# ayildiri/polymer-chemprop

Hardware: AMD Instinct MI355X
Metric: edges/sec MPN forward, batch=64 polymer graphs, depth=3 hidden=300 (higher is better)
Workload: dtype fp32; 1 GPU; MPNEncoder.forward on synthetic polymer batches of 64 graphs (avg E=6164 directed edges), depth=3, hidden=300, 8 resident batches cycled per rank; global_batch=64, depth=3, hidden=300, parallelism=dp1 (independent graphs, no collective in the forward), streams=3

## Files before the change

polymer-chemprop_amd/csrc/common.hpp:

```cpp
#pragma once
#include <hip/hip_runtime.h>
#include <stdint.h>

#include <type_traits>

namespace wd {

typedef float floatx16 __attribute__((ext_vector_type(16)));

enum Act : int { ACT_RELU = 0, ACT_LEAKY = 1, ACT_PRELU = 2, ACT_TANH = 3, ACT_SELU = 4, ACT_ELU = 5,
                 ACT_IDENTITY = 6 };

constexpr float SELU_ALPHA = 1.6732632423543772848170429916717f;
constexpr float SELU_SCALE = 1.0507009873554804934193349852946f;

__device__ __forceinline__ float act_fwd(int act, float z, float slope) {
    switch (act) {
    case ACT_RELU: return z < 0.f ? 0.f : z;
    case ACT_LEAKY: return z > 0.f ? z : 0.1f * z;
    case ACT_PRELU: return z > 0.f ? z : slope * z;
    case ACT_TANH: return tanhf(z);
    case ACT_SELU: return z > 0.f ? SELU_SCALE * z : SELU_SCALE * (SELU_ALPHA * expm1f(z));
    case ACT_ELU: return z > 0.f ? z : expm1f(z);
    default: return z;
// ... 37 lines not shown
    }
}

__device__ __forceinline__ float dropout_scale(uint64_t seed, uint32_t layer, uint32_t row, uint32_t col, float p) {
    uint64_t x = seed ^ (0x9E3779B97F4A7C15ull * (uint64_t)(layer + 1));
    x ^= ((uint64_t)row << 32) | col;
    x += 0x9E3779B97F4A7C15ull;
    x = (x ^ (x >> 30)) * 0xBF58476D1CE4E5B9ull;
    x = (x ^ (x >> 27)) * 0x94D049BB133111EBull;
    x ^= x >> 31;
    const float u = (float)(uint32_t)(x >> 40) * (1.0f / 16777216.0f);
    return u >= p ? 1.0f / (1.0f - p) : 0.0f;
}

#ifndef WD_STAMPS
#define WD_STAMPS 0
#endif
#if WD_STAMPS
constexpr int WD_STAMP_SLOTS = 16, WD_STAMP_WG = 8192;
__device__ uint64_t g_wd_stamps[WD_STAMP_WG * WD_STAMP_SLOTS];
__device__ __forceinline__ void wd_stamp(int slot) {
    const uint64_t t = __builtin_amdgcn_s_memrealtime();
    if (threadIdx.x == 0 && blockIdx.x < WD_STAMP_WG)
        __hip_atomic_store(&g_wd_stamps[blockIdx.x * WD_STAMP_SLOTS + slot], t, __ATOMIC_RELAXED, __HIP_MEMORY_SCOPE_AGENT);
}
constexpr int WD_LSTAMP_WG = 512;
__device__ uint64_t g_wd_lstamps[WD_LSTAMP_WG * 16 * 8];
__device__ uint64_t g_wd_estamps[WD_STAMP_WG * 8];
__device__ __forceinline__ void wd_estamp(int slot) {
    const uint64_t t = __builtin_amdgcn_s_memrealtime();
    if (threadIdx.x == 0 && blockIdx.x < WD_STAMP_WG)
        __hip_atomic_store(&g_wd_estamps[blockIdx.x * 8 + slot], t, __ATOMIC_RELAXED, __HIP_MEMORY_SCOPE_AGENT);
}
__device__ __forceinline__ void wd_lstamp(int chunk, int slot) {
    const uint64_t t = __builtin_amdgcn_s_memtime();
    if ((threadIdx.x & 63) == 0 && blockIdx.x < WD_LSTAMP_WG && chunk < 16)
        __hip_atomic_store(&g_wd_lstamps[(blockIdx.x * 16 + chunk) * 8 + slot], t, __ATOMIC_RELAXED, __HIP_MEMORY_SCOPE_AGENT);
}
#else
__device__ __forceinline__ void wd_stamp(int) {}
__device__ __forceinline__ void wd_estamp(int) {}
__device__ __forceinline__ void wd_lstamp(int, int) {}
#endif

__device__ __forceinline__ float4 f4zero() { return make_float4(0.f, 0.f, 0.f, 0.f); }

__device__ __forceinline__ void fma4(float4 &acc, float c, const float4 &v) {
    acc.x = fmaf(c, v.x, acc.x);
    acc.y = fmaf(c, v.y, acc.y);
    acc.z = fmaf(c, v.z, acc.z);
    acc.w = fmaf(c, v.w, acc.w);
}

__device__ __forceinline__ float4 ld4(const float *p) { return *reinterpret_cast<const float4 *>(p); }
__device__ __forceinline__ void st4(float *p, const float4 &v) { *reinterpret_cast<float4 *>(p) = v; }

__device__ __forceinline__ int xcd_tile(int b, int ntiles) {
    const int base = ntiles >> 3, rem = ntiles & 7;
    const int x = b & 7, local = b >> 3;
    return x * base + (x < rem ? x : rem) + local;
}

constexpr int WD_MULTI = 8;
template <typename T, int NJ = WD_MULTI> struct Multi {
    T p[NJ];
    int t0[NJ + 1];
    int n;
};
template <typename T, int NJ>
__device__ __forceinline__ const T &multi_pick(const Multi<T, NJ> &M, int g, int &tile) {
    int j = 0;
    while (j + 1 < M.n && g >= M.t0[j + 1]) ++j;
    tile = g - M.t0[j];
    return M.p[j];
// ... 4 lines not shown
```

polymer-chemprop_amd/csrc/fused_mp.hpp:

```cpp
#pragma once
#include "gemm_x6.hpp"
#include "kernels.hpp"
#include "wdmpnn.h"

namespace wd {


constexpr int BLK_BONDS = 128, BLK_ATOMS = 64;
constexpr int BLK_MOLS = 64;
constexpr int ELLW = 8;
static_assert(ELLW % 4 == 0, "ELL rows of whole 4-byte index words and float4 weight groups");

struct EllRow {
    uint32_t ix[ELLW / 4];
    float w[ELLW];
};
__device__ __forceinline__ EllRow ell_zero() {
    EllRow e;
    for (int k = 0; k < ELLW / 4; ++k) e.ix[k] = 0;
    for (int k = 0; k < ELLW; ++k) e.w[k] = 0.f;
    return e;
}
__device__ __forceinline__ EllRow ell_load(const uint8_t *idx, const float *coef, size_t row) {
    EllRow e;
// ... 676 lines not shown
            const int v = tid + NT * u, lb = v / U8, c = 8 * (v % U8);
            if (lb >= ((B.bn + 15) & ~15)) break;
            h2_store8(prs, h2_blk_off<BLK_BONDS>(lb, n0 + c), BLK_BONDS * 64, ym[u][0], ym[u][1], s);
        }
        wd_estamp(7);
    } else {
        publish_max(mx, P.amax + (size_t)blk * P.n_tiles + nt, red);
    }
    if constexpr (EO_LAST) {
        __syncthreads();
        eo_half();
    }
}

constexpr int WO_MAXK = 160;

struct WoReadoutP {
    const uint8_t *fa; int kpa; int kca;
    int kcw;
    const uint8_t *ag; int kp;
    const uint8_t *wo;
    const float *bias;
    const int32_t *blocks;
    const float *w_atoms; const int32_t *mol_start, *mol_size; const float *xn;
    int agg; float norm; const float *zero_vec;
    int act; const float *slope; float p_drop; uint64_t seed; uint32_t layer;
    float *out; int ncols;
    int n_tiles;
    const float *eo;
    int Hk, ldeo;
    float *zosave;
    const uint8_t *apairs; const uint32_t *a_amax; int a_nw, a_g;
    const uint8_t *woh; const uint32_t *wo_amax;
};

template <int BN> struct WoWaves;
template <> struct WoWaves<64> { static constexpr int WM = 4, WN = 2; };
template <> struct WoWaves<80> { static constexpr int WM = 2, WN = 5; };

template <int BN, int CPS, int NJ = WD_MULTI, bool PAIRS = false>
__global__ __launch_bounds__(PAIRS ? 512 : 64 * WoWaves<BN>::WM * WoWaves<BN>::WN, PAIRS ? 4 : 1) void wo_readout_kernel(const Multi<WoReadoutP, NJ> MP) {
    constexpr int BM = BLK_ATOMS, LDC = BN + 4, WM = PAIRS ? 4 : WoWaves<BN>::WM, WN = PAIRS ? 1 : WoWaves<BN>::WN;
    constexpr int NT = PAIRS ? 512 : 64 * WM * WN;
    constexpr int WS = 2;
    constexpr int EPI_BYTES = (BM * LDC + BM + 3 * BLK_MOLS + BN) * 4;
    constexpr int LDS_BYTES = PAIRS ? (h2p_lds_bytes<BM, BN>() > EPI_BYTES ? h2p_lds_bytes<BM, BN>() : EPI_BYTES)
                                    : WS * CPS * x6_stage_bytes<BM, BN>();
    __shared__ __attribute__((aligned(16))) uint8_t lds[LDS_BYTES];
    int tile;
    const WoReadoutP &P = multi_pick(MP, xcd_tile(blockIdx.x, gridDim.x), tile);
    const int blk = tile / P.n_tiles, nt = tile % P.n_tiles, n0 = nt * BN;
    BlockRow B = PAIRS ? BlockRow{} : load_block(P.blocks, blk);
    const int tid = threadIdx.x;
    X6Operands O{};
    O.a0 = P.fa; O.nkc0 = P.kpa >> 5; O.kc0 = P.kca;
    O.a1 = P.ag; O.nkc1 = P.kp >> 5; O.kc1 = P.kp >> 5;
    O.rb = blk;
    O.a_rows = B.an;
    O.b = P.wo + ((size_t)nt * (P.kcw + (P.kp >> 5)) + (P.kcw - P.kca)) * (3 * BN * 64);
    constexpr int C4 = BN / 4;
    static_assert((PAIRS || NT % C4 == 0) && BM <= NT, "one bias group per thread, one atom weight per thread");
    int nm = min(B.mh - B.ml, BLK_MOLS);
    if (P.zosave && blk == 0 && tid < BN / 4) st4(P.zosave + n0 + 4 * tid, f4zero());
    float4 bb = f4zero();
    float watom = 0.f, mxn = 0.f;
    int mstart = 0, msize = 0;
    constexpr int EPU = (BM * C4 + NT - 1) / NT;
    float4 eo[EPU];
    auto prefetch = [&](int phase) {
        if (phase != 0) return;
        if (!PAIRS || tid < C4) bb = ld4(P.bias + n0 + 4 * (tid % C4));
        if (tid < B.an) watom = P.w_atoms[B.as + tid];
#pragma unroll
        for (int j = 0; j < EPU; ++j) {
            const int v = tid + NT * j, la = v / C4, c = 4 * (v % C4);
            eo[j] = P.eo && v < BM * C4 && la < B.an ? ld4(P.eo + (size_t)(B.as + la) * P.ldeo + n0 + c) : f4zero();
        }
        if (tid < nm) {
            mstart = P.mol_start[B.ml + tid];
            msize = P.mol_size[B.ml + tid];
            mxn = P.xn[B.ml + tid];
        }
    };
    float *H = reinterpret_cast<float *>(lds);
    floatx4 acc[BM / WM / 16][BN / WN / 16];
    if constexpr (PAIRS) {
        auto rows = [&]() {
            B = load_block(P.blocks, blk);
            nm = min(B.mh - B.ml, BLK_MOLS);
            prefetch(0);
            return B.an;
        };
        uint32_t wom = 0;
        auto words = [&]() {
            wom = *P.wo_amax;
            return lane_word(P.a_amax + (size_t)blk * P.a_nw, P.a_nw);
        };
        int se;
        h2_mainloop_pairs<BM, BN>(P.apairs + (size_t)blk * (P.kp >> 5) * (2 * BM * 64),
                                  P.woh + (size_t)nt * (P.kp >> 5) * (2 * BN * 64), P.kp >> 5, rows, words, P.a_g, lds,
                                  acc, se);
        __syncthreads();
        if (threadIdx.x < 256)
            x6_acc_to_lds_scaled<BM, BN, 4, 1>(acc, H, se >= 0 ? __uint_as_float((uint32_t)(254 - se) << 23) : 1.f,
                                               h2_inv_scale(wom));
    } else {
        x6_mainloop<BM, BN, WM, WN, WS, CPS>(O, lds, acc, prefetch);
        __syncthreads();
        x6_acc_to_lds<BM, BN, WM, WN>(acc, H);
    }
    float *Wl = H + BM * LDC;
    float *Ml = Wl + BM;
    static_assert(EPI_BYTES <= LDS_BYTES, "readout staging fits");
    static_assert(BLK_MOLS <= NT, "one molecule per thread in the prefetch");
    if (tid < BM) Wl[tid] = watom;
    if (PAIRS && tid < C4) st4(Ml + 3 * BLK_MOLS + 4 * tid, bb);
    if (tid < nm) {
        Ml[tid] = __int_as_float(mstart);
        Ml[BLK_MOLS + tid] = __int_as_float(msize);
        Ml[2 * BLK_MOLS + tid] = mxn;
    }
    __syncthreads();
    with_act(P.act, [&](auto act_c) {
        constexpr int ACT = decltype(act_c)::value;
        const float slope = ACT == ACT_PRELU ? P.slope[0] : 0.f;
#pragma unroll
        for (int j = 0; j < EPU; ++j) {
            const int v = tid + NT * j;
            if (v >= BM * C4) break;
            const int la = v / C4, c = 4 * (v % C4);
            float4 hv = ld4(H + la * LDC + c);
            hv.x += eo[j].x; hv.y += eo[j].y; hv.z += eo[j].z; hv.w += eo[j].w;
            const float4 b4 = PAIRS ? ld4(Ml + 3 * BLK_MOLS + c) : bb;
            float z[4] = {hv.x + b4.x, hv.y + b4.y, hv.z + b4.z, hv.w + b4.w};
            if (P.zosave && la < B.an) st4(P.zosave + (size_t)(B.as + la) * P.Hk + n0 + c, make_float4(z[0], z[1], z[2], z[3]));
#pragma unroll
            for (int q = 0; q < 4; ++q) z[q] = act_fwd(ACT, z[q], slope);
            if (P.p_drop > 0.f && la < B.an)
#pragma unroll
                for (int q = 0; q < 4; ++q) z[q] *= dropout_scale(P.seed, P.layer, B.as + la, n0 + c + q, P.p_drop);
            st4(H + la * LDC + c, make_float4(z[0], z[1], z[2], z[3]));
        }
    });
    __syncthreads();
    constexpr int RP = 8;
    static_assert(NT % RP == 0 && 64 % RP == 0, "lane groups stay inside a wave");
    for (int t = tid; t < nm * BN * RP; t += NT) {
        const int part = t % RP, u = t / RP, im = u / BN, i = B.ml + im, cc = u % BN, col = n0 + cc;
        const int n = __float_as_int(Ml[BLK_MOLS + im]);
        float s = 0.f, wsum = 0.f;
        const int a0 = __float_as_int(Ml[im]) - B.as;
        for (int a = part; a < n; a += RP) {
            const float w = Wl[a0 + a];
            s = fmaf(w, H[(a0 + a) * LDC + cc], s);
            wsum += w;
        }
#pragma unroll
        for (int off = 1; off < RP; off <<= 1) {
            s += __shfl_xor(s, off, 64);
            wsum += __shfl_xor(wsum, off, 64);
        }
        if (part != 0 || col >= P.ncols) continue;
        float v;
        if (n == 0) {
            v = P.zero_vec[col];
        } else {
            const float m = P.agg == 0 ? s / wsum : (P.agg == 2 ? s / P.norm : s);
            v = Ml[2 * BLK_MOLS + im] * m;
        }
        P.out[(size_t)i * P.ncols + col] = v;
    }
}

}
```

polymer-chemprop_amd/csrc/gemm_x6.hpp:

```cpp
#pragma once
#include "gemm.hpp"
#include "planes.hpp"

#include <type_traits>

namespace wd {

#ifndef WD_STAMP_GEMM
#define WD_STAMP_GEMM 0
#endif

struct X6Params {
    const float *a0; int lda0; int ka0;
    const float *a1; int lda1; int ka1;
    const float *bf; int ldb;
    int M, N;
    int tiles_m, tiles_n;
    Epi epi;
    const uint32_t *a_words; int a_cv;
    const uint32_t *b_word;
};

template <int BM, int BK, bool H2 = false>
__global__ __launch_bounds__(4 * BM) void gemm_x6_kernel(X6Params P) {
// ... 796 lines not shown
        if (kc + H2_B_AHEAD < nchunks) issue_b(kc + H2_B_AHEAD);
        const uint8_t *st = lds + (kc % NA) * ASTAGE, *sb = lds + NA * ASTAGE + (kc % NB) * BSTAGE;
        dispatch_upto<TM>(na, [&](auto c) { compute_n(st, sb, c); });
        if (WD_STAMPS && wave == 0) {
            asm volatile("s_waitcnt lgkmcnt(0)" ::: "memory");
            wd_lstamp(kc, 3);
        }
    }
    __builtin_amdgcn_s_waitcnt(0x0070);
}

#ifndef WD_H2P_STAGES
#define WD_H2P_STAGES 3
#endif
constexpr int H2P_STAGES = WD_H2P_STAGES;
template <int BM, int BN>
constexpr int h2p_stage_bytes() { return 2 * BM * 64 + 2 * BN * 64; }
template <int BM, int BN>
constexpr int h2p_lds_bytes() { return H2P_STAGES * h2p_stage_bytes<BM, BN>(); }

#ifndef WD_H2P_FRAG
#define WD_H2P_FRAG 0
#endif
#ifndef WD_H2P_EARLY
#define WD_H2P_EARLY 0
#endif
#ifndef WD_H2P_UNIFORM
#define WD_H2P_UNIFORM 1
#endif
struct NoLoaderHook {
    __device__ void issue() {}
    __device__ void finish() {}
};
template <int BM, int BN, int FRAG = WD_H2P_FRAG, typename Rows, typename Words, typename LoaderHook = NoLoaderHook>
__device__ __forceinline__ void h2_mainloop_pairs(const uint8_t *a_src, const uint8_t *b_src, int nchunks, Rows &&rows,
                                                  Words &&words, int G, uint8_t *lds, floatx4 (&acc)[BM / 64][BN / 16],
                                                  int &se_out, LoaderHook &&lhook = LoaderHook()) {
    constexpr bool EARLY = WD_H2P_EARLY;
    static_assert(BM == 128 || BM == 64, "four consumer waves of BM / 4 rows");
    constexpr int RW = BM / 4, TM = RW / 16, TN = BN / 16;
    constexpr int APL = BM * 64, BPL = BN * 64, STAGE = h2p_stage_bytes<BM, BN>(), NS = H2P_STAGES;
    constexpr int AP = 2 * BM / 16, APW = AP / 4;
    constexpr int BP = 2 * BN / 16, BPW = (BP + 3) / 4;
    static_assert(AP % 4 == 0, "A pieces split evenly over the loader waves");
    const int tid = threadIdx.x, lane = tid & 63, wave = WD_H2P_UNIFORM ? __builtin_amdgcn_readfirstlane(tid >> 6) : tid >> 6, w4 = wave & 3;
    const int g = lane >> 4, i16 = lane & 15;
    const int roff = (NS - (nchunks - 1) % NS) % NS;
#pragma unroll
    for (int a = 0; a < TM; ++a)
#pragma unroll
        for (int b = 0; b < TN; ++b) acc[a][b] = floatx4{0.f, 0.f, 0.f, 0.f};
    if (wave >= 4) {
        int src[APW + BPW], dst[APW + BPW];
#pragma unroll
        for (int j = 0; j < APW; ++j) {
            const int c = 4 * j + w4, q = 64 * c + lane, p = q / (BM * 4), r = (q >> 2) % BM, sl = q & 3;
            src[j] = p * APL + r * 64 + 16 * (sl ^ ((r >> 1) & 3));
            dst[j] = 1024 * c;
        }
#pragma unroll
        for (int j = 0; j < BPW; ++j) {
            const int c = 4 * j + w4, q = 64 * c + lane, p = (q / (BN * 4)) % 2, r = (q >> 2) % BN, sl = q & 3;
            src[APW + j] = p * BPL + r * 64 + 16 * (sl ^ ((r >> 1) & 3));
            dst[APW + j] = 2 * APL + 1024 * c;
        }
        auto issue = [&](int kc, const bool (&on)[APW + BPW]) {
            uint8_t *st = lds + ((kc + roff) % NS) * STAGE;
            const uint8_t *ablk = a_src + (size_t)kc * (2 * APL), *bblk = b_src + (size_t)kc * (2 * BPL);
#pragma unroll
            for (int j = 0; j < APW; ++j)
                if (on[j]) glds16_untracked(ablk + src[j], st + dst[j]);
#pragma unroll
            for (int j = 0; j < BPW; ++j)
                if (on[APW + j]) glds16_untracked(bblk + src[APW + j], st + dst[APW + j]);
        };
        bool all[APW + BPW], on[APW + BPW];
#pragma unroll
        for (int j = 0; j < APW; ++j) all[j] = true;
#pragma unroll
        for (int j = 0; j < BPW; ++j) all[APW + j] = BP % 4 == 0 || 4 * j + w4 < BP;
        if constexpr (EARLY) {
#pragma unroll
            for (int c = 0; c < NS - 1; ++c)
                if (c < nchunks) issue(c, all);
            __builtin_amdgcn_sched_barrier(0);
        }
        const int a_rows = rows();
        int mine = 0;
#pragma unroll
        for (int j = 0; j < APW; ++j) {
            on[j] = 16 * ((4 * j + w4) % (BM / 16)) < a_rows;
            mine += on[j];
        }
#pragma unroll
        for (int j = 0; j < BPW; ++j) {
            on[APW + j] = all[APW + j];
            mine += on[APW + j];
        }
        mine = __builtin_amdgcn_readfirstlane(mine);
        if constexpr (!EARLY) {
#pragma unroll
            for (int c = 0; c < NS - 1; ++c)
                if (c < nchunks) issue(c, on);
        }
        lhook.issue();
        dispatch_upto<APW + BPW>(mine, [&](auto m_c) {
            constexpr int M = decltype(m_c)::value;
            for (int kc = 0; kc < nchunks; ++kc) {
                if (WD_STAMPS && wave == 4) wd_lstamp(kc, 4);
                if (nchunks - 1 - kc >= NS - 2) asm volatile("s_waitcnt vmcnt(%0)" ::"n"((NS - 2) * M) : "memory");
                else wait_vmcnt((nchunks - 1 - kc) * M);
                if (WD_STAMPS && wave == 4) wd_lstamp(kc, 5);
                __builtin_amdgcn_s_barrier();
                if (kc + NS - 1 < nchunks) issue(kc + NS - 1, on);
            }
        });
        __builtin_amdgcn_s_waitcnt(0x0070);
        lhook.finish();
        se_out = -1;
        return;
    }
    const int a_rows = rows();
    const uint32_t wv = words();
    int ao[TM], bo[TN];
#pragma unroll
    for (int a = 0; a < TM; ++a) ao[a] = x6_slot(RW * w4 + 16 * a + i16, g);
#pragma unroll
    for (int b = 0; b < TN; ++b) bo[b] = x6_slot(16 * b + i16, g);
    const int na = min(TM, max(0, (a_rows - RW * w4 + 15) >> 4));
    constexpr int BIG = 1 << 20;
    const int k0 = min((32 * lane) / G, 63), k1 = min((32 * lane + 16) / G, 63);
    const uint32_t lw0 = (uint32_t)__shfl((int)wv, k0, 64), lw1 = (uint32_t)__shfl((int)wv, k1, 64);
    const int s0 = lw0 ? h2_sexp(lw0) : BIG, s1 = lw1 ? h2_sexp(lw1) : BIG;
    const int cur = BIG - (int)wave_max_u32((uint32_t)(BIG - (lane < nchunks ? min(s0, s1) : BIG)));
    auto f16code = [&](int se) -> uint32_t {
        const int d = se - cur;
        return d > 24 ? 0u : (uint32_t)__builtin_bit_cast(unsigned short, (_Float16)__builtin_amdgcn_ldexpf(1.0f, -d));
    };
    const uint32_t fcode = f16code(s0) | (f16code(s1) << 16);
    const int fsh = lane < 32 ? 0 : 16;
    auto compute_n = [&](const uint8_t *st, const uint8_t *sb, auto na_c, _Float16 fl) {
        constexpr int NA = decltype(na_c)::value;
        constexpr int SCH = FRAG & 3, NB = SCH == 2 ? TN : 2;
        f16x8 af[TM][2], bq[NB][2];
#pragma unroll
        for (int p = 0; p < 2; ++p) {
#pragma unroll
            for (int a = 0; a < NA; ++a) {
                af[a][p] = *reinterpret_cast<const f16x8 *>(st + p * APL + ao[a]);
                af[a][p] = af[a][p] * fl;
            }
#pragma unroll
            for (int b = 0; b < (SCH == 2 ? TN : 1); ++b) bq[b][p] = *reinterpret_cast<const f16x8 *>(sb + p * BPL + bo[b]);
        }
#pragma unroll
        for (int b = 0; b < TN; ++b) {
            const int cb = SCH == 2 ? b : (b & 1);
            if constexpr (SCH == 1) {
                if (b + 1 < TN)
#pragma unroll
                    for (int p = 0; p < 2; ++p) bq[(b + 1) & 1][p] = *reinterpret_cast<const f16x8 *>(sb + p * BPL + bo[b + 1]);
                __builtin_amdgcn_sched_barrier(0);
// ... 106 lines not shown
```

polymer-chemprop_amd/csrc/wdmpnn.hip:

```cpp
#include <hip/hip_runtime.h>

#include <algorithm>
#include <array>
#include <cstdarg>
#include <cstdio>
#include <cstdlib>
#include <cmath>
#include <cstring>
#include <string>
#include <vector>

#include "feed.hpp"
#include "fused_mp.hpp"
#include "gemm.hpp"
#include "gemm_x6.hpp"
#include "graph_build.hpp"
#include "kernels.hpp"
#include "selfcheck.hpp"
#include "small_fwd.hpp"
#include "wdmpnn.h"

using namespace wd;

namespace {
// ... 14 lines not shown
#define WD_KERNELS_OK() WD_TRY(self_check_once())

#define WD_CHECK_LAUNCH(what)                                                                  \
    do {                                                                                       \
        hipError_t e_ = hipGetLastError();                                                     \
        if (e_ != hipSuccess) return fail(-(int)e_, "%s: %s", what, hipGetErrorString(e_));   \
    } while (0)
#define WD_TRY(x)             \
    do {                      \
        int rc_ = (x);        \
        if (rc_) return rc_;  \
    } while (0)

struct SelfCheck {
    int rc;
    std::string why;
    int n_host, n_dev;
};
const SelfCheck &self_check_result() {
    static const SelfCheck r = [] {
        SelfCheck c{};
        c.rc = code_object_check(reinterpret_cast<const void *>(&self_check_result), c.why, c.n_host, c.n_dev);
        return c;
    }();
    return r;
}
int self_check_once() {
    const SelfCheck &c = self_check_result();
    return c.rc ? fail(WD_ERR_UNSUPPORTED, "libwdmpnn self-check: %s", c.why.c_str()) : 0;
}

#ifndef WD_WO_PAIRS
#define WD_WO_PAIRS 1
#endif

#ifndef WD_FEED_EVENT_SYNC
#define WD_FEED_EVENT_SYNC hipEventBlockingSync
#endif

#ifndef WD_BWD_H2
#define WD_BWD_H2 1
#endif

inline int rup(int x, int m) { return (x + m - 1) / m * m; }


inline size_t align256(size_t x) { return (x + 255) & ~size_t(255); }
bool aligned16(const void *p) { return ((uintptr_t)p & 15) == 0; }

int ew_blocks(size_t total) {
    size_t b = (total + 255) / 256;
    if (b > 4096) b = 4096;
    if (b < 1) b = 1;
    return (int)b;
}

struct Variant {
    bool f32;
    bool one_launch;
    bool staged;
    bool pairs;
    bool pair_tiles;
    int stop;
    bool wo_dump;
};
Variant decode_variant(int v) {
// ... 645 lines not shown
    L.mol_start = take((size_t)c->n_mols * 4 + 4);
    L.mol_size = take((size_t)c->n_mols * 4 + 4);
    L.xn = take((size_t)c->n_mols * 4 + 4);
    L.b2revb = take((size_t)c->n_bonds * 4);
    L.blocks = take((size_t)c->n_blocks * 32 + 32);
    L.bond_blk_row = take((size_t)L.Rbp * 4);
    L.atom_blk_row = take((size_t)L.Vap * 4);
    L.bond_src_blk = take((size_t)L.Rbp);
    L.bond_tail = take((size_t)L.Rbp * 2);
    L.msg_ell_idx = take((size_t)L.Rbp * GB_ELLW);
    L.msg_ell_coef = take((size_t)L.Rbp * GB_ELLW * 4);
    L.agg_ell_idx = take((size_t)L.Vap * GB_ELLW);
    L.agg_ell_coef = take((size_t)L.Vap * GB_ELLW * 4);
    const int rows[4] = {c->n_bonds, c->n_atoms, c->n_bonds, c->n_bonds};
    const int nnz[4] = {c->nnz_msg, c->nnz_agg, c->nnz_msg, c->nnz_agg};
    for (int q = 0; q < 4; ++q) {
        L.csr[q][0] = take((size_t)(rows[q] + 1) * 4);
        L.csr[q][1] = take((size_t)(nnz[q] + GB_CSR_PAD) * 4);
        L.csr[q][2] = take((size_t)(nnz[q] + GB_CSR_PAD) * 4);
    }
    L.total = off;
    return 0;
}

struct FusedJob {
    const WdGraph *g;
    Dims D;
    FwdLayout L;
    char *ws;
    float *out;
};

template <typename T, typename Fill>
int launch_multi(const FusedJob *jobs, int n, int tiles_per_blk, Fill &&fill, Multi<T> &M) {
    M = Multi<T>{};
    M.n = n;
    int t = 0;
    for (int j = 0; j < n; ++j) {
        M.t0[j] = t;
        fill(M.p[j], jobs[j]);
        t += jobs[j].D.nblk * tiles_per_blk;
    }
    for (int j = n; j <= WD_MULTI; ++j) M.t0[j] = t;
    return t;
}
template <typename T>
Multi<T, 1> one_job(const Multi<T> &M) {
    Multi<T, 1> o{};
    o.p[0] = M.p[0]; o.t0[0] = M.t0[0]; o.t0[1] = M.t0[1]; o.n = 1;
    return o;
}
template <typename T, typename Launch>
void with_jobs(int n, const Multi<T> &M, Launch &&launch) {
    if (n == 1) launch(one_job(M), std::integral_constant<int, 1>{});
    else launch(M, std::integral_constant<int, WD_MULTI>{});
}

struct FusedCtx {
    const FusedJob *jobs;
    int n;
    const WdParams *p;
    const WdConfig *c;
    const PackLayout &PL;
    const char *pk;
    hipStream_t st;
    const Dims &D0;
    int Hk, BN;
    const float *W(size_t off) const { return (const float *)(pk + off); }
    static float *F(const FusedJob &J, size_t off) { return (float *)(J.ws + off); }
    static uint32_t *slot(const FusedJob &J, int t) { return (uint32_t *)(J.ws + J.L.amax[t & 1]); }
};

int fused_input(const FusedCtx &X) {
    const Dims &D0 = X.D0;
// ... 97 lines not shown
            Q.apairs = last && D0.wo_pairs ? (uint8_t *)(J.ws + J.L.Ab) : nullptr;
            Q.amax_out = X.slot(J, t);
        }
    }, M);
    auto go = [&](auto bn_c, auto last_c) {
        constexpr int BNc = decltype(bn_c)::value;
        constexpr bool LAST = decltype(last_c)::value;
        host_with_act(X.c->activation, [&](auto act_c) {
            constexpr int A = decltype(act_c)::value;
            if (D0.atom)
                hipLaunchKernelGGL((mp_layer_kernel<BNc, LAST, A, true, 1>), dim3(grid), dim3(MP_THREADS), 0, X.st, one_job(M));
            else with_jobs(X.n, M, [&](const auto &Mn, auto nj) {
                constexpr int NJ = decltype(nj)::value;
                if (BNc != 80 || !pairs)
                    hipLaunchKernelGGL((mp_layer_kernel<BNc, LAST, A, false, NJ>), dim3(grid), dim3(MP_THREADS), 0, X.st, Mn);
                else if constexpr (BNc == 80)
                    hipLaunchKernelGGL((mp_layer_kernel<BNc, LAST, A, false, NJ, true>), dim3(grid), dim3(MP_THREADS), 0, X.st, Mn);
            });
        });
    };
    using I80 = std::integral_constant<int, 80>;
    using I64 = std::integral_constant<int, 64>;
    if (BN == 80) { if (last) go(I80{}, std::true_type{}); else go(I80{}, std::false_type{}); }
    else { if (last) go(I64{}, std::true_type{}); else go(I64{}, std::false_type{}); }
    WD_CHECK_LAUNCH("mp_layer");
    return 0;
}

int fused_wo_readout(const FusedCtx &X) {
    const Dims &D0 = X.D0;
    const PackLayout &PL = X.PL;
    const int Hk = X.Hk, BN = X.BN;
    Multi<WoReadoutP> M;
    const int grid = launch_multi(X.jobs, X.n, Hk / BN, [&](WoReadoutP &R, const FusedJob &J) {
        const WdGraph *g = J.g;
        R.fa = g->f_atoms_blk_x6 ? (const uint8_t *)g->f_atoms_blk_x6 : (const uint8_t *)(J.ws + J.L.Ab);
        R.kpa = g->ld_atoms; R.kcw = J.D.Fak / 32;
        R.kca = D0.codes || J.D.atom ? 0 : R.kcw;
        R.eo = D0.codes ? X.F(J, J.L.Eo) : (J.D.atom ? X.F(J, J.L.In3) + 2 * Hk : nullptr); R.Hk = Hk;
        R.ldeo = J.D.atom ? 3 * Hk : Hk;
        R.ag = (const uint8_t *)(J.ws + J.L.Ab); R.kp = Hk;
        R.wo = (const uint8_t *)(X.pk + (BN == 80 ? PL.WoX80 : PL.WoX)); R.bias = X.W(PL.bo);
        R.blocks = g->blocks;
        R.w_atoms = g->w_atoms; R.mol_start = g->mol_start; R.mol_size = g->mol_size; R.xn = g->degree_of_polym;
        R.agg = X.c->aggregation; R.norm = X.c->aggregation_norm; R.zero_vec = X.p->zero_vec;
        R.act = X.c->activation; R.slope = X.p->prelu; R.p_drop = X.c->dropout; R.seed = X.c->seed; R.layer = J.D.T;
        R.out = J.out; R.ncols = J.D.H; R.n_tiles = Hk / BN;
        R.zosave = J.D.save ? X.F(J, J.L.Zo) : nullptr;
        if (D0.V.wo_dump && J.D.T == 3)
            R.zosave = D0.lay_pairs ? X.F(J, J.L.Mp[1]) : X.F(J, J.L.Zb[1]);
        if (D0.wo_pairs) {
            R.apairs = (const uint8_t *)(J.ws + J.L.Ab); R.a_amax = X.slot(J, J.D.T - 1); R.a_nw = Hk / BN; R.a_g = BN;
            R.woh = (const uint8_t *)(X.pk + PL.WoH); R.wo_amax = (const uint32_t *)(X.pk + PL.wo_amax) + 64;
        }
    }, M);
    if (grid <= 0) return 0;
    with_jobs(X.n, M, [&](const auto &Mn, auto nj) {
        constexpr int NJ = decltype(nj)::value;
        if (D0.wo_pairs)
            hipLaunchKernelGGL((wo_readout_kernel<80, 1, NJ, true>), dim3(grid), dim3(512), 0, X.st, Mn);
        else if (BN == 80)
            hipLaunchKernelGGL((wo_readout_kernel<80, NJ == 1 ? 1 : 2, NJ>), dim3(grid), dim3(64 * WoWaves<80>::WM * WoWaves<80>::WN), 0, X.st, Mn);
        else
            hipLaunchKernelGGL((wo_readout_kernel<64, 1, NJ>), dim3(grid), dim3(64 * WoWaves<64>::WM * WoWaves<64>::WN), 0, X.st, Mn);
    });
    WD_CHECK_LAUNCH("wo_readout");
    return 0;
}

int fused_forward(const FusedJob *jobs, int n, const WdParams *p, const WdConfig *c, const PackLayout &PL,
                  const char *pk, hipStream_t st) {
    if (n < 1 || n > WD_MULTI) return fail(WD_ERR_ARG, "fused forward: %d jobs per launch (1..%d)", n, WD_MULTI);
    const Dims &D0 = jobs[0].D;
    if (D0.atom && n > 1)
        return fail(WD_ERR_UNSUPPORTED, "fused forward: atom messages run one batch per launch");
    for (int j = 1; j < n; ++j) {
        const Dims &D = jobs[j].D;
        if (D.codes != D0.codes || D.Hk != D0.Hk || D.T != D0.T || D.atom != D0.atom || D.Fa != D0.Fa ||
            D.Fb != D0.Fb || D.save != D0.save || D.pairs != D0.pairs)
            return fail(WD_ERR_UNSUPPORTED, "fused forward: batches of one launch differ in layout");
    }
    const FusedCtx X{jobs, n, p, c, PL, pk, st, D0, D0.Hk, D0.bn};
    const int stop = D0.V.stop;
    WD_TRY(fused_input(X));
    if (D0.codes && stop == 1) return 0;
    for (int t = 1; t < D0.T; ++t) {
        if (t == 1) WD_TRY(record_prof(c, 0, 0, st));
        WD_TRY(fused_layer(X, t));
        if (t == D0.T - 1) WD_TRY(record_prof(c, 0, 1, st));
        if (stop == t + 1) return 0;
    }
    return fused_wo_readout(X);
// ... 35 lines not shown
int wdmpnn_abi_version(void) { return WDMPNN_ABI_VERSION; }

int wdmpnn_self_check(int32_t *n_host_kernels, int32_t *n_device_kernels) {
    const SelfCheck &c = self_check_result();
    if (n_host_kernels) *n_host_kernels = c.n_host;
    if (n_device_kernels) *n_device_kernels = c.n_dev;
    return self_check_once();
}

int wdmpnn_debug_fwd_offsets(const WdGraph *g, const WdParams *p, const WdConfig *c, size_t *out) {
    Dims D;
    WD_TRY(get_dims(g, p, c, D));
    const FwdLayout L = fwd_layout(D, p->packed == nullptr);
    const PackLayout PL = pack_layout(D);
    const size_t v[15] = {L.Z.empty() ? 0 : L.Z[0], L.Mp[0], L.Mp[1], L.Ab, L.amax[0], L.amax[1], L.Zb[0], L.Zb[1],
                          L.total, (size_t)D.pairs, PL.WoH, PL.wo_amax, PL.WhH, PL.amax, L.Eo};
    memcpy(out, v, sizeof(v));
    return 0;
}

int wdmpnn_debug_stamps(void *host, size_t bytes) {
#if WD_STAMPS
    if (hipDeviceSynchronize() != hipSuccess) return fail(WD_ERR_ARG, "sync");
    if (hipMemcpyFromSymbol(host, HIP_SYMBOL(g_wd_stamps), std::min(bytes, sizeof(g_wd_stamps))) != hipSuccess)
        return fail(WD_ERR_ARG, "stamps copy");
    if (bytes > sizeof(g_wd_stamps) &&
        hipMemcpyFromSymbol((char *)host + sizeof(g_wd_stamps), HIP_SYMBOL(g_wd_lstamps),
                            std::min(bytes - sizeof(g_wd_stamps), sizeof(g_wd_lstamps))) != hipSuccess)
        return fail(WD_ERR_ARG, "loop stamps copy");
    const size_t eo = sizeof(g_wd_stamps) + sizeof(g_wd_lstamps);
    if (bytes > eo && hipMemcpyFromSymbol((char *)host + eo, HIP_SYMBOL(g_wd_estamps),
                                          std::min(bytes - eo, sizeof(g_wd_estamps))) != hipSuccess)
        return fail(WD_ERR_ARG, "embed stamps copy");
    return 0;
#else
    (void)host; (void)bytes;
    return fail(WD_ERR_UNSUPPORTED, "library built without WD_STAMPS");
#endif
}



const char *wdmpnn_last_error(void) { return g_err.c_str(); }

int wdmpnn_packed_params_bytes(const WdGraph *g, const WdParams *p, const WdConfig *c, size_t *bytes) {
    Dims D;
    WD_TRY(get_dims(g, p, c, D));
    if (!bytes) return fail(WD_ERR_ARG, "null bytes");
    *bytes = pack_layout(D).total;
    return 0;
}

int wdmpnn_pack_params(const WdGraph *g, const WdParams *p, const WdConfig *c, void *packed, size_t bytes,
                       void *stream) {
    WD_KERNELS_OK();
    Dims D;
    WD_TRY(get_dims(g, p, c, D));
    if (!packed || bytes < pack_layout(D).total) return fail(WD_ERR_WORKSPACE, "packed buffer too small");
    return pack_params(D, p, (char *)packed, (hipStream_t)stream);
}

int wdmpnn_workspace_bytes(const WdGraph *g, const WdParams *p, const WdConfig *c, size_t *bytes) {
    Dims D;
    WD_TRY(get_dims(g, p, c, D));
    if (!bytes) return fail(WD_ERR_ARG, "null bytes");
    *bytes = fwd_layout(D, p->packed == nullptr).total;
// ... 1047 lines not shown
```

Before: 243.0 million edges/s.

## Process two atom blocks per workgroup in W_o readout pairs kernel

Adds a wo_readout_pair_kernel in which each 512-thread workgroup handles two consecutive 64-atom blocks (BM=128) against one W_o column tile. The shared pairs mainloop gains a SPLIT mode that loads the two blocks from separate A regions. The aim is to halve the grid and reuse each W_o tile load across twice as many rows, which cuts B-operand traffic and per-workgroup overhead. It is enabled by default when a launch carries multiple jobs, and it disables the EARLY prefetch path. Timing stamps (compiled out by default) are also added.

```diff
diff --git a/polymer-chemprop_amd/csrc/common.hpp b/polymer-chemprop_amd/csrc/common.hpp
--- a/polymer-chemprop_amd/csrc/common.hpp
+++ b/polymer-chemprop_amd/csrc/common.hpp
@@ -93,6 +93,12 @@
     if (threadIdx.x == 0 && blockIdx.x < WD_STAMP_WG)
         __hip_atomic_store(&g_wd_estamps[blockIdx.x * 8 + slot], t, __ATOMIC_RELAXED, __HIP_MEMORY_SCOPE_AGENT);
 }
+__device__ uint64_t g_wd_wstamps[WD_STAMP_WG * 8];
+__device__ __forceinline__ void wd_wstamp(int slot) {
+    const uint64_t t = __builtin_amdgcn_s_memrealtime();
+    if (threadIdx.x == 0 && blockIdx.x < WD_STAMP_WG)
+        __hip_atomic_store(&g_wd_wstamps[blockIdx.x * 8 + slot], t, __ATOMIC_RELAXED, __HIP_MEMORY_SCOPE_AGENT);
+}
 __device__ __forceinline__ void wd_lstamp(int chunk, int slot) {
     const uint64_t t = __builtin_amdgcn_s_memtime();
     if ((threadIdx.x & 63) == 0 && blockIdx.x < WD_LSTAMP_WG && chunk < 16)
@@ -101,6 +107,7 @@
 #else
 __device__ __forceinline__ void wd_stamp(int) {}
 __device__ __forceinline__ void wd_estamp(int) {}
+__device__ __forceinline__ void wd_wstamp(int) {}
 __device__ __forceinline__ void wd_lstamp(int, int) {}
 #endif
 
diff --git a/polymer-chemprop_amd/csrc/fused_mp.hpp b/polymer-chemprop_amd/csrc/fused_mp.hpp
--- a/polymer-chemprop_amd/csrc/fused_mp.hpp
+++ b/polymer-chemprop_amd/csrc/fused_mp.hpp
@@ -732,6 +732,7 @@
     float *zosave;
     const uint8_t *apairs; const uint32_t *a_amax; int a_nw, a_g;
     const uint8_t *woh; const uint32_t *wo_amax;
+    int nblk;
 };
 
 template <int BN> struct WoWaves;
@@ -748,6 +749,7 @@
                                     : WS * CPS * x6_stage_bytes<BM, BN>();
     __shared__ __attribute__((aligned(16))) uint8_t lds[LDS_BYTES];
     int tile;
+    if (PAIRS) wd_wstamp(0);
     const WoReadoutP &P = multi_pick(MP, xcd_tile(blockIdx.x, gridDim.x), tile);
     const int blk = tile / P.n_tiles, nt = tile % P.n_tiles, n0 = nt * BN;
     BlockRow B = PAIRS ? BlockRow{} : load_block(P.blocks, blk);
@@ -797,10 +799,13 @@
             return lane_word(P.a_amax + (size_t)blk * P.a_nw, P.a_nw);
         };
         int se;
+        wd_wstamp(1);
         h2_mainloop_pairs<BM, BN>(P.apairs + (size_t)blk * (P.kp >> 5) * (2 * BM * 64),
                                   P.woh + (size_t)nt * (P.kp >> 5) * (2 * BN * 64), P.kp >> 5, rows, words, P.a_g, lds,
                                   acc, se);
+        wd_wstamp(2);
         __syncthreads();
+        wd_wstamp(3);
         if (threadIdx.x < 256)
             x6_acc_to_lds_scaled<BM, BN, 4, 1>(acc, H, se >= 0 ? __uint_as_float((uint32_t)(254 - se) << 23) : 1.f,
                                                h2_inv_scale(wom));
@@ -821,6 +826,7 @@
         Ml[2 * BLK_MOLS + tid] = mxn;
     }
     __syncthreads();
+    if (PAIRS) wd_wstamp(4);
     with_act(P.act, [&](auto act_c) {
         constexpr int ACT = decltype(act_c)::value;
         const float slope = ACT == ACT_PRELU ? P.slope[0] : 0.f;
@@ -843,6 +849,7 @@
         }
     });
     __syncthreads();
+    if (PAIRS) wd_wstamp(5);
     constexpr int RP = 8;
     static_assert(NT % RP == 0 && 64 % RP == 0, "lane groups stay inside a wave");
     for (int t = tid; t < nm * BN * RP; t += NT) {
@@ -870,6 +877,144 @@
         }
         P.out[(size_t)i * P.ncols + col] = v;
     }
+    if (PAIRS) wd_wstamp(6);
 }
 
+template <int BN, int NJ = WD_MULTI>
+__global__ __launch_bounds__(512, 4) void wo_readout_pair_kernel(const Multi<WoReadoutP, NJ> MP) {
+    constexpr int BM = 2 * BLK_ATOMS, LDC = BN + 4, NT = 512, C4 = BN / 4;
+    constexpr int EPI_BYTES = (BM * LDC + BM + 2 * 3 * BLK_MOLS + BN) * 4;
+    constexpr int LDS_BYTES = h2p_lds_bytes<BM, BN>() > EPI_BYTES ? h2p_lds_bytes<BM, BN>() : EPI_BYTES;
+    static_assert(LDS_BYTES <= 80 * 1024, "two workgroups per CU");
+    static_assert(BLK_MOLS <= BLK_ATOMS && BM <= NT, "one atom weight and one molecule per thread in the prefetch");
+    __shared__ __attribute__((aligned(16))) uint8_t lds[LDS_BYTES];
+    int tile;
+    wd_wstamp(0);
+    const WoReadoutP &P = multi_pick(MP, xcd_tile(blockIdx.x, gridDim.x), tile);
+    const int blk0 = 2 * (tile / P.n_tiles), nt = tile % P.n_tiles, n0 = nt * BN;
+    const bool two = blk0 + 1 < P.nblk;
+    const int tid = threadIdx.x;
+    const int hi = (tid >> 6) & 1, li = tid & 63;
+    BlockRow B[2] = {BlockRow{}, BlockRow{}};
+    int nm[2] = {0, 0};
+    if (P.zosave && blk0 == 0 && tid < C4) st4(P.zosave + n0 + 4 * tid, f4zero());
+    float4 bb = f4zero();
+    float watom = 0.f, mxn = 0.f;
+    int mstart = 0, msize = 0;
+    constexpr int EPU = BM * C4 / NT;
+    static_assert(BM * C4 % NT == 0, "whole epilogue units per thread");
+    float4 eo[EPU];
+    auto rows = [&]() {
+        B[0] = load_block(P.blocks, blk0);
+        B[1] = load_block(P.blocks, two ? blk0 + 1 : blk0);
+        if (!two) B[1].an = 0, B[1].mh = B[1].ml;
+        nm[0] = min(B[0].mh - B[0].ml, BLK_MOLS);
+        nm[1] = min(B[1].mh - B[1].ml, BLK_MOLS);
+        if (tid < C4) bb = ld4(P.bias + n0 + 4 * tid);
+        if (tid < BM) {
+            const int as = hi ? B[1].as : B[0].as, an = hi ? B[1].an : B[0].an;
+            const int ml = hi ? B[1].ml : B[0].ml, n = hi ? nm[1] : nm[0];
+            if (li < an) watom = P.w_atoms[as + li];
+            if (li < n) {
+                mstart = P.mol_start[ml + li];
+                msize = P.mol_size[ml + li];
+                mxn = P.xn[ml + li];
+            }
+        }
+#pragma unroll
+        for (int j = 0; j < EPU; ++j) {
+            const int v = tid + NT * j, r = v / C4, c = 4 * (v % C4), la = r & 63;
+            const int as = r < 64 ? B[0].as : B[1].as, an = r < 64 ? B[0].an : B[1].an;
+            eo[j] = P.eo && la < an ? ld4(P.eo + (size_t)(as + la) * P.ldeo + n0 + c) : f4zero();
+        }
+        return make_int2(B[0].an, B[1].an);
+    };
+    uint32_t wom = 0;
+    auto words = [&]() {
+        wom = *P.wo_amax;
+        const bool second = __builtin_amdgcn_readfirstlane(tid >> 6) >= 2;
+        return lane_word(P.a_amax + (size_t)(second && two ? blk0 + 1 : blk0) * P.a_nw, second && !two ? 0 : P.a_nw);
+    };
+    float *H = reinterpret_cast<float *>(lds);
+    floatx4 acc[BM / 64][BN / 16];
+    int se;
+    wd_wstamp(1);
+    h2_mainloop_pairs<BM, BN, WD_H2P_FRAG, true>(P.apairs + (size_t)blk0 * (P.kp >> 5) * (2 * BLK_ATOMS * 64),
+                                                 P.woh + (size_t)nt * (P.kp >> 5) * (2 * BN * 64), P.kp >> 5, rows, words,
+                                                 P.a_g, lds, acc, se);
+    wd_wstamp(2);
+    __syncthreads();
+    wd_wstamp(3);
+    if (tid < 256)
+        x6_acc_to_lds_scaled<BM, BN, 4, 1>(acc, H, se >= 0 ? __uint_as_float((uint32_t)(254 - se) << 23) : 1.f,
+                                           h2_inv_scale(wom));
+    float *Wl = H + BM * LDC;
+    float *Ml = Wl + BM;
+    float *Bl = Ml + 2 * 3 * BLK_MOLS;
+    if (tid < BM) {
+        Wl[tid] = watom;
+        if (li < (hi ? nm[1] : nm[0])) {
+            float *Mh = Ml + hi * 3 * BLK_MOLS;
+            Mh[li] = __int_as_float(mstart);
+            Mh[BLK_MOLS + li] = __int_as_float(msize);
+            Mh[2 * BLK_MOLS + li] = mxn;
+        }
+    }
+    if (tid < C4) st4(Bl + 4 * tid, bb);
+    __syncthreads();
+    wd_wstamp(4);
+    with_act(P.act, [&](auto act_c) {
+        constexpr int ACT = decltype(act_c)::value;
+        const float slope = ACT == ACT_PRELU ? P.slope[0] : 0.f;
+#pragma unroll
+        for (int j = 0; j < EPU; ++j) {
+            const int v = tid + NT * j, r = v / C4, c = 4 * (v % C4), la = r & 63;
+            const int as = r < 64 ? B[0].as : B[1].as, an = r < 64 ? B[0].an : B[1].an;
+            float4 hv = ld4(H + r * LDC + c);
+            hv.x += eo[j].x; hv.y += eo[j].y; hv.z += eo[j].z; hv.w += eo[j].w;
+            const float4 b4 = ld4(Bl + c);
+            float z[4] = {hv.x + b4.x, hv.y + b4.y, hv.z + b4.z, hv.w + b4.w};
+            if (P.zosave && la < an) st4(P.zosave + (size_t)(as + la) * P.Hk + n0 + c, make_float4(z[0], z[1], z[2], z[3]));
+#pragma unroll
+            for (int q = 0; q < 4; ++q) z[q] = act_fwd(ACT, z[q], slope);
+            if (P.p_drop > 0.f && la < an)
+#pragma unroll
+                for (int q = 0; q < 4; ++q) z[q] *= dropout_scale(P.seed, P.layer, as + la, n0 + c + q, P.p_drop);
+            st4(H + r * LDC + c, make_float4(z[0], z[1], z[2], z[3]));
+        }
+    });
+    __syncthreads();
+    wd_wstamp(5);
+    constexpr int RP = 8;
+    static_assert(NT % RP == 0 && 64 % RP == 0, "lane groups stay inside a wave");
+    for (int t = tid; t < (nm[0] + nm[1]) * BN * RP; t += NT) {
+        const int part = t % RP, u = t / RP, im = u / BN, cc = u % BN, col = n0 + cc;
+        const int h = im >= nm[0], il = im - (h ? nm[0] : 0), i = (h ? B[1].ml : B[0].ml) + il;
+        const float *Mh = Ml + h * 3 * BLK_MOLS;
+        const int n = __float_as_int(Mh[BLK_MOLS + il]);
+        float s = 0.f, wsum = 0.f;
+        const int a0 = __float_as_int(Mh[il]) - (h ? B[1].as : B[0].as) + BLK_ATOMS * h;
+        for (int a = part; a < n; a += RP) {
+            const float w = Wl[a0 + a];
+            s = fmaf(w, H[(a0 + a) * LDC + cc], s);
+            wsum += w;
+        }
+#pragma unroll
+        for (int off = 1; off < RP; off <<= 1) {
+            s += __shfl_xor(s, off, 64);
+            wsum += __shfl_xor(wsum, off, 64);
+        }
+        if (part != 0 || col >= P.ncols) continue;
+        float v;
+        if (n == 0) {
+            v = P.zero_vec[col];
+        } else {
+            const float m = P.agg == 0 ? s / wsum : (P.agg == 2 ? s / P.norm : s);
+            v = Mh[2 * BLK_MOLS + il] * m;
+        }
+        P.out[(size_t)i * P.ncols + col] = v;
+    }
+    wd_wstamp(6);
 }
+
+}
diff --git a/polymer-chemprop_amd/csrc/gemm_x6.hpp b/polymer-chemprop_amd/csrc/gemm_x6.hpp
--- a/polymer-chemprop_amd/csrc/gemm_x6.hpp
+++ b/polymer-chemprop_amd/csrc/gemm_x6.hpp
@@ -852,14 +852,17 @@
     __device__ void issue() {}
     __device__ void finish() {}
 };
-template <int BM, int BN, int FRAG = WD_H2P_FRAG, typename Rows, typename Words, typename LoaderHook = NoLoaderHook>
+template <int BM, int BN, int FRAG = WD_H2P_FRAG, bool SPLIT = false, typename Rows, typename Words,
+          typename LoaderHook = NoLoaderHook>
 __device__ __forceinline__ void h2_mainloop_pairs(const uint8_t *a_src, const uint8_t *b_src, int nchunks, Rows &&rows,
                                                   Words &&words, int G, uint8_t *lds, floatx4 (&acc)[BM / 64][BN / 16],
                                                   int &se_out, LoaderHook &&lhook = LoaderHook()) {
-    constexpr bool EARLY = WD_H2P_EARLY;
+    constexpr bool EARLY = WD_H2P_EARLY && !SPLIT;
+    static_assert(!SPLIT || BM == 128, "two 64-row blocks");
     static_assert(BM == 128 || BM == 64, "four consumer waves of BM / 4 rows");
     constexpr int RW = BM / 4, TM = RW / 16, TN = BN / 16;
     constexpr int APL = BM * 64, BPL = BN * 64, STAGE = h2p_stage_bytes<BM, BN>(), NS = H2P_STAGES;
+    constexpr int SPL = SPLIT ? 64 * 64 : APL;
     constexpr int AP = 2 * BM / 16, APW = AP / 4;
     constexpr int BP = 2 * BN / 16, BPW = (BP + 3) / 4;
     static_assert(AP % 4 == 0, "A pieces split evenly over the loader waves");
@@ -875,7 +878,8 @@
 #pragma unroll
         for (int j = 0; j < APW; ++j) {
             const int c = 4 * j + w4, q = 64 * c + lane, p = q / (BM * 4), r = (q >> 2) % BM, sl = q & 3;
-            src[j] = p * APL + r * 64 + 16 * (sl ^ ((r >> 1) & 3));
+            if constexpr (SPLIT) src[j] = (r >> 6) * nchunks * (2 * SPL) + p * SPL + (r & 63) * 64 + 16 * (sl ^ ((r >> 1) & 3));
+            else src[j] = p * APL + r * 64 + 16 * (sl ^ ((r >> 1) & 3));
             dst[j] = 1024 * c;
         }
 #pragma unroll
@@ -886,7 +890,7 @@
         }
         auto issue = [&](int kc, const bool (&on)[APW + BPW]) {
             uint8_t *st = lds + ((kc + roff) % NS) * STAGE;
-            const uint8_t *ablk = a_src + (size_t)kc * (2 * APL), *bblk = b_src + (size_t)kc * (2 * BPL);
+            const uint8_t *ablk = a_src + (size_t)kc * (2 * SPL), *bblk = b_src + (size_t)kc * (2 * BPL);
 #pragma unroll
             for (int j = 0; j < APW; ++j)
                 if (on[j]) glds16_untracked(ablk + src[j], st + dst[j]);
@@ -905,11 +909,13 @@
                 if (c < nchunks) issue(c, all);
             __builtin_amdgcn_sched_barrier(0);
         }
-        const int a_rows = rows();
+        const auto a_rows = rows();
         int mine = 0;
 #pragma unroll
         for (int j = 0; j < APW; ++j) {
-            on[j] = 16 * ((4 * j + w4) % (BM / 16)) < a_rows;
+            const int grp = (4 * j + w4) % (BM / 16);
+            if constexpr (SPLIT) on[j] = 16 * (grp & 3) < (grp < 4 ? a_rows.x : a_rows.y);
+            else on[j] = 16 * grp < a_rows;
             mine += on[j];
         }
 #pragma unroll
@@ -940,14 +946,21 @@
         se_out = -1;
         return;
     }
-    const int a_rows = rows();
+    int a_rows, row0 = RW * w4;
+    if constexpr (SPLIT) {
+        const auto ar = rows();
+        a_rows = w4 < 2 ? ar.x : ar.y;
+        row0 = RW * (w4 & 1);
+    } else {
+        a_rows = rows();
+    }
     const uint32_t wv = words();
     int ao[TM], bo[TN];
 #pragma unroll
     for (int a = 0; a < TM; ++a) ao[a] = x6_slot(RW * w4 + 16 * a + i16, g);
 #pragma unroll
     for (int b = 0; b < TN; ++b) bo[b] = x6_slot(16 * b + i16, g);
-    const int na = min(TM, max(0, (a_rows - RW * w4 + 15) >> 4));
+    const int na = min(TM, max(0, (a_rows - row0 + 15) >> 4));
     constexpr int BIG = 1 << 20;
     const int k0 = min((32 * lane) / G, 63), k1 = min((32 * lane + 16) / G, 63);
     const uint32_t lw0 = (uint32_t)__shfl((int)wv, k0, 64), lw1 = (uint32_t)__shfl((int)wv, k1, 64);
diff --git a/polymer-chemprop_amd/csrc/wdmpnn.hip b/polymer-chemprop_amd/csrc/wdmpnn.hip
--- a/polymer-chemprop_amd/csrc/wdmpnn.hip
+++ b/polymer-chemprop_amd/csrc/wdmpnn.hip
@@ -70,6 +70,9 @@
 
 #ifndef WD_WO_PAIRS
 #define WD_WO_PAIRS 1
+#endif
+#ifndef WD_WO_BLOCK_PAIRS
+#define WD_WO_BLOCK_PAIRS 1
 #endif
 
 #ifndef WD_FEED_EVENT_SYNC
@@ -781,14 +784,14 @@
 };
 
 template <typename T, typename Fill>
-int launch_multi(const FusedJob *jobs, int n, int tiles_per_blk, Fill &&fill, Multi<T> &M) {
+int launch_multi(const FusedJob *jobs, int n, int tiles_per_blk, Fill &&fill, Multi<T> &M, int blks_per_wg = 1) {
     M = Multi<T>{};
     M.n = n;
     int t = 0;
     for (int j = 0; j < n; ++j) {
         M.t0[j] = t;
         fill(M.p[j], jobs[j]);
-        t += jobs[j].D.nblk * tiles_per_blk;
+        t += (jobs[j].D.nblk + blks_per_wg - 1) / blks_per_wg * tiles_per_blk;
     }
     for (int j = n; j <= WD_MULTI; ++j) M.t0[j] = t;
     return t;
@@ -952,8 +955,10 @@
     const PackLayout &PL = X.PL;
     const int Hk = X.Hk, BN = X.BN;
     Multi<WoReadoutP> M;
+    const bool blk_pairs = D0.wo_pairs && (WD_WO_BLOCK_PAIRS == 2 || (WD_WO_BLOCK_PAIRS == 1 && X.n > 1));
     const int grid = launch_multi(X.jobs, X.n, Hk / BN, [&](WoReadoutP &R, const FusedJob &J) {
         const WdGraph *g = J.g;
+        R.nblk = J.D.nblk;
         R.fa = g->f_atoms_blk_x6 ? (const uint8_t *)g->f_atoms_blk_x6 : (const uint8_t *)(J.ws + J.L.Ab);
         R.kpa = g->ld_atoms; R.kcw = J.D.Fak / 32;
         R.kca = D0.codes || J.D.atom ? 0 : R.kcw;
@@ -973,11 +978,13 @@
             R.apairs = (const uint8_t *)(J.ws + J.L.Ab); R.a_amax = X.slot(J, J.D.T - 1); R.a_nw = Hk / BN; R.a_g = BN;
             R.woh = (const uint8_t *)(X.pk + PL.WoH); R.wo_amax = (const uint32_t *)(X.pk + PL.wo_amax) + 64;
         }
-    }, M);
+    }, M, blk_pairs ? 2 : 1);
     if (grid <= 0) return 0;
     with_jobs(X.n, M, [&](const auto &Mn, auto nj) {
         constexpr int NJ = decltype(nj)::value;
-        if (D0.wo_pairs)
+        if (blk_pairs)
+            hipLaunchKernelGGL((wo_readout_pair_kernel<80, NJ>), dim3(grid), dim3(512), 0, X.st, Mn);
+        else if (D0.wo_pairs)
             hipLaunchKernelGGL((wo_readout_kernel<80, 1, NJ, true>), dim3(grid), dim3(512), 0, X.st, Mn);
         else if (BN == 80)
             hipLaunchKernelGGL((wo_readout_kernel<80, NJ == 1 ? 1 : 2, NJ>), dim3(grid), dim3(64 * WoWaves<80>::WM * WoWaves<80>::WN), 0, X.st, Mn);
@@ -1079,6 +1086,10 @@
     if (bytes > eo && hipMemcpyFromSymbol((char *)host + eo, HIP_SYMBOL(g_wd_estamps),
                                           std::min(bytes - eo, sizeof(g_wd_estamps))) != hipSuccess)
         return fail(WD_ERR_ARG, "embed stamps copy");
+    const size_t wo = eo + sizeof(g_wd_estamps);
+    if (bytes > wo && hipMemcpyFromSymbol((char *)host + wo, HIP_SYMBOL(g_wd_wstamps),
+                                          std::min(bytes - wo, sizeof(g_wd_wstamps))) != hipSuccess)
+        return fail(WD_ERR_ARG, "W_o stamps copy");
     return 0;
 #else
     (void)host; (void)bytes;
```

Result: no change. 241.4 million edges/s (-0.7%).
